# inai17ibar/video-diffusion-pipeline-parallel

Hardware: AMD Instinct MI355X
Metric: steady-state videos/sec (whole node), SVD 14f x 25step (higher is better)
Workload: dtype f16

## Files before the change

### include/svdpipe.h

```cpp
#ifndef SVDPIPE_H
#define SVDPIPE_H

#include <stddef.h>
#include <stdint.h>

#ifdef __cplusplus
extern "C" {
#endif

#define SP_OK 0
#define SP_EINVAL (-1)
#define SP_ELAUNCH (-2)

const char *sp_last_error(void);
int sp_version(void);
#define SP_ZERO_PAGE_BYTES 4096

enum { SP_A_LINEAR = 0, SP_A_CONV3X3 = 1, SP_A_TEMPORAL3 = 2 };

typedef struct sp_gemm_desc {
  const void *a;
  int64_t lda;
  int mode;
  int cin;
// ... 20 lines not shown
  float euler_sigma, euler_sigma_next;
  int euler_frames; int64_t euler_hw;
  void *workspace; size_t workspace_bytes;
  float *ln_out; float ln_out_eps;
  int64_t w_group_rows; int64_t w_group_stride;
  float *gn_part;
  const void *a2; int64_t lda2; int cin2;
  int64_t euler_guidance_ld;
} sp_gemm_desc;

int sp_gemm_f16(const sp_gemm_desc *desc, void *stream);
size_t sp_gemm_desc_size(void);
size_t sp_gemm_workspace_bytes(const sp_gemm_desc *desc);

const char *sp_gemm_last_kernel(void);

int sp_gemm_set_route(int route, int bm, int bn);

int sp_gemv_f16(const void *x, int64_t ldx, const void *w, const float *b, float *y, void *y_f16,
                int64_t ldy, int rows, int n, int k, int silu_in, int silu_out, void *stream);
int sp_gemv_batched_f16(const void *x, int64_t ldx, int64_t x_stride, const void *w, int64_t w_stride,
                        const float *b, int64_t b_stride, float *y, void *y_f16, int64_t ldy, int64_t y_stride,
                        int batch, int rows, int n, int k, int silu_in, int silu_out, void *stream);

int sp_sinusoid_f16(const float *values, void *out, int count, int dim, void *stream);

size_t sp_groupnorm_ws_bytes(int instances, int64_t rows, int c, int groups);
int sp_groupnorm_f16(const void *x, const float *gamma, const float *beta, void *y, int instances,
                     int64_t rows, int c, int groups, float eps, int fuse_silu, void *ws,
                     size_t ws_bytes, void *stream);
// ... 107 lines not shown
```

### video-diffusion-pipeline-parallel_amd/csrc/gemm.hip

```cpp
#include <cstring>
#include "gemm_args.h"
#include <stdlib.h>

using namespace spgemm;

namespace {


template <int BM, int BN, int WM, int WN, int STAGES>
__global__ __launch_bounds__(WM *WN * 64, 2) void gemm_f16_kernel(const GemmArgs p) {
  constexpr int NW = WM * WN;
  constexpr int THREADS = NW * 64;
  constexpr int WTM = BM / WM, WTN = BN / WN;
  constexpr int TN = WTN / 16;
  constexpr int TM = WTM / 16;
  constexpr int A_BYTES = BM * BK * 2;
  constexpr int B_BYTES = BN * BK * 2;
  constexpr int STAGE = A_BYTES + B_BYTES;
  constexpr int A_LOADS = BM / 8 / NW;
  constexpr int B_LOADS = BN / 8 / NW;
  constexpr int L = A_LOADS + B_LOADS;
  static_assert(A_LOADS * 8 * NW == BM && B_LOADS * 8 * NW == BN, "tile rows must split evenly over waves");
  static_assert(STAGES == 2 || STAGES == 3, "2- or 3-deep ring");
  extern __shared__ __attribute__((aligned(16))) char smem[];
// ... 568 lines not shown
}

extern "C" int sp_gemm_f32out_f16(const void *a_, int64_t lda, const void *w, void *d, int m, int n, int k,
                                  const void *zero_page, void *stream) {
  SP_REQUIRE(a_ && w && d && zero_page, "sp_gemm_f32out_f16: null a/w/d/zero_page");
  SP_REQUIRE(m > 0 && n > 0 && n % 256 == 0, "sp_gemm_f32out_f16: n=%d must be a positive multiple of 256 (m=%d)", n, m);
  SP_REQUIRE(k >= 64 && k % 64 == 0, "sp_gemm_f32out_f16: k=%d must be a multiple of 64", k);
  SP_REQUIRE(lda >= k && lda % 8 == 0, "sp_gemm_f32out_f16: lda=%lld invalid", (long long)lda);
  SP_REQUIRE(((uintptr_t)d & 15) == 0, "sp_gemm_f32out_f16: d must be 16-byte aligned");
  GemmArgs a{};
  a.a = (const f16 *)a_; a.w = (const f16 *)w; a.zero = (const char *)zero_page;
  a.lda = lda; a.mode = SP_A_LINEAR; a.cin = k; a.taps = 1; a.m = m; a.n = n; a.k = k;
  a.oscale = 1.0f; a.bias2_rows = m; a.ldb2 = n;
  a.ksplit = 1; a.partial = (float *)d;
  return spgemm::launch_pp(a, 256, 256, (hipStream_t)stream);
}

extern "C" int sp_gemm_f16(const sp_gemm_desc *d, void *stream) {
  SP_REQUIRE(d != nullptr, "sp_gemm_f16: null descriptor");
  SP_REQUIRE(d->a && d->w && d->d && d->zero_page, "sp_gemm_f16: null a/w/d/zero_page");
  SP_REQUIRE(d->m > 0 && d->n > 0, "sp_gemm_f16: m,n must be positive (m=%d n=%d)", d->m, d->n);
  SP_REQUIRE(d->cin > 0 && d->cin % 64 == 0, "sp_gemm_f16: cin=%d must be a multiple of 64", d->cin);
  SP_REQUIRE(d->n % 64 == 0, "sp_gemm_f16: n=%d must be a multiple of 64", d->n);
  SP_REQUIRE(d->mode >= SP_A_LINEAR && d->mode <= SP_A_TEMPORAL3, "sp_gemm_f16: bad mode %d", d->mode);
  SP_REQUIRE(d->lda >= d->cin && d->lda % 8 == 0, "sp_gemm_f16: lda=%lld invalid", (long long)d->lda);
  const int nout_cols = d->geglu ? d->n / 2 : d->n;
  SP_REQUIRE(d->n_store >= 0 && d->n_store <= nout_cols, "sp_gemm_f16: n_store=%d must be 0 (all) or 1 ... %d output columns",
             d->n_store, nout_cols);
  const int stored_cols = d->n_store > 0 ? d->n_store : nout_cols;
  SP_REQUIRE(d->ldd >= stored_cols && (d->ldd % 8 == 0 || (d->n_store > 0 && d->n_store < 8)),
// ... 120 lines not shown
```

### video-diffusion-pipeline-parallel_amd/csrc/gemm_args.h

```cpp
#pragma once
#include "common.h"

namespace spgemm {

constexpr int BK = 64;

template <int N>
__device__ __forceinline__ void wait_vm_lgkm() {
  asm volatile("s_waitcnt vmcnt(%0) lgkmcnt(0)" ::"n"(N) : "memory");
}

struct GemmArgs {
  const f16 *a;
  const f16 *a2;
  int64_t lda2;
  int cin2;
  const f16 *w;
  const float *bias;
  const float *bias2;
  const f16 *res1;
  const f16 *res2;
  const f16 *eul_lat; f16 *eul_out; const f16 *eul_u; const float *eul_gs;
  int64_t eul_ldu, eul_hw, eul_ldg;
  int eul_frames;
// ... 7 lines not shown
  f16 *d;
  const char *zero;
  int64_t lda, ldr1, ldr2, ldd, hw, bias2_rows, ldb2;
  int64_t w_group_rows, w_group_stride;
  int mode, cin, taps;
  int n_img, hin, win, hout, wout, stride, ups;
  int frames;
  int m, n, k;
  float oscale, r1scale, r2scale;
  int geglu, n_store;
  int tiles_m, tiles_n;
  int ksplit;
  float *partial;
  int dbg;
  int stagger;
};

__device__ __forceinline__ int xcd_remap(int bid, int nwg) {
  const int q = nwg >> 3, r = nwg & 7;
  const int xcd = bid & 7;
  const int base = xcd < r ? xcd * (q + 1) : r * (q + 1) + (xcd - r) * q;
  return base + (bid >> 3);
}


void note_kernel(const char *fmt, ...);
void note_kernel_suffix(const char *suffix);

int launch_pp(GemmArgs &a, int bm, int bn, hipStream_t s);

bool ps_supported(const GemmArgs &a, int bm, int bn);
int launch_ps(GemmArgs &a, int bm, int bn, hipStream_t s);

}
```

### video-diffusion-pipeline-parallel_amd/csrc/gemm_pp.hip

```cpp
#include "gemm_args.h"
#include <stdlib.h>
#include <type_traits>

namespace spgemm {
namespace {

constexpr int PBK = 32, PNW = 8;


#ifdef SP_GEMM_EXPERIMENTS
constexpr int PP_TRACE_WGS = 16384, PP_TRACE_SLOTS = 12;
__device__ long long g_pp_trace[PP_TRACE_WGS * PP_TRACE_SLOTS];
#define PP_TRACE(slot)                                                                              \
  do {                                                                                              \
    if (threadIdx.x == 0 && blockIdx.x < PP_TRACE_WGS)                                              \
      g_pp_trace[blockIdx.x * PP_TRACE_SLOTS + (slot)] = wall_clock64();                            \
  } while (0)
#define PP_TRACE_CLK(slot)                                                                          \
  do {                                                                                              \
    if (threadIdx.x == 0 && blockIdx.x < PP_TRACE_WGS)                                              \
      g_pp_trace[blockIdx.x * PP_TRACE_SLOTS + (slot)] = (long long)__builtin_amdgcn_s_memtime();   \
  } while (0)
#else
#define PP_TRACE(slot) do {} while (0)
// ... 7 lines not shown
#endif
constexpr int pp_stages(int bm, int bn) { return bm == 128 ? 3 : (bm == 192 && bn == 256 ? SP_PP_STAGES_192_256 : 4); }

template <int N>
__device__ __forceinline__ void wait_vm() { asm volatile("s_waitcnt vmcnt(%0)" ::"n"(N) : "memory"); }

template <int L>
__device__ __forceinline__ void wait_dma(int ksteps_left) {
  if (ksteps_left >= 3) wait_vm<3 * L>();
  else if (ksteps_left == 2) wait_vm<2 * L>();
  else if (ksteps_left == 1) wait_vm<L>();
  else wait_vm<0>();
}

#define WROWS_OF(pbm, wtm) ((pbm) / (wtm))
template <int PBM, int BN, int TN, int TM, int WTN, int WTM, bool GEGLU, int NT, bool GNRES = false>
__device__ __forceinline__ void pp_epilogue(const GemmArgs &p, f32x4 (&acc)[TN][TM], char *smem, int tile_m,
                                            int tile_n, int wm, int wn, int tid, int fr, int fq) {
  constexpr int bno = GEGLU ? BN / 2 : BN;
  constexpr int cpr = bno >> 3;
  constexpr int TNO = GEGLU ? TN / 2 : TN;
  constexpr int NCH = PBM * cpr, ITERS = (NCH + NT - 1) / NT, ITERS_A = ITERS / 2;
  static_assert(cpr % 8 == 0, "chunk swizzle works on aligned groups of 8 chunks");
  const int ncols_total = GEGLU ? p.n / 2 : p.n;
  const int nstore = p.n_store > 0 ? p.n_store : ncols_total;
  const int64_t mbase = (int64_t)tile_m * PBM;

  auto res_src = [&](const f16 *res, int64_t ldr, int it) -> const f16 * {
    const int idx = tid + it * NT;
    const int r = idx / cpr, c = idx - r * cpr;
    const int64_t m = mbase + r;
    const int col = tile_n * bno + c * 8;
    const bool ok = idx < NCH && m < p.m && col + 8 <= nstore;
// ... 16 lines not shown
      if (p.bias) b = *(const f32x4 *)(p.bias + n);
#pragma unroll
      for (int j = 0; j < TM; ++j) acc[i][j] = (acc[i][j] - st[j][0] * cs) * st[j][1] + b;
      __builtin_amdgcn_sched_barrier(0);
    }
  }
  if constexpr (!GEGLU) {
    if (p.gn_part && !p.res1 && !p.res2) {
      auto row16_sum = [](float v) {
        v += __builtin_bit_cast(float, __builtin_amdgcn_mov_dpp(__builtin_bit_cast(int, v), 0xB1, 0xF, 0xF, true));
        v += __builtin_bit_cast(float, __builtin_amdgcn_mov_dpp(__builtin_bit_cast(int, v), 0x4E, 0xF, 0xF, true));
        v += __builtin_bit_cast(float, __builtin_amdgcn_mov_dpp(__builtin_bit_cast(int, v), 0x141, 0xF, 0xF, true));
        v += __builtin_bit_cast(float, __builtin_amdgcn_mov_dpp(__builtin_bit_cast(int, v), 0x140, 0xF, 0xF, true));
        return v;
      };
      float *dst = p.gn_part + (((int64_t)tile_m * WROWS_OF(PBM, WTM) + wm) * p.n + (int64_t)tile_n * BN + wn * WTN) * 2;
#pragma unroll
      for (int i = 0; i < TN; ++i) {
        f32x4 sm = {0.f, 0.f, 0.f, 0.f}, sq = {0.f, 0.f, 0.f, 0.f};
#pragma unroll
        for (int j = 0; j < TM; ++j) {
          const f32x4 v = acc[i][j] * p.oscale;
          sm += v;
          sq += v * v;
        }
#pragma unroll
        for (int r = 0; r < 4; ++r) { sm[r] = row16_sum(sm[r]); sq[r] = row16_sum(sq[r]); }
        if (fr == 0) {
          float *o = dst + (i * 16 + 4 * fq) * 2;
          *(f32x4 *)o = (f32x4){sm[0], sq[0], sm[1], sq[1]};
          *(f32x4 *)(o + 4) = (f32x4){sm[2], sq[2], sm[3], sq[3]};
// ... 91 lines not shown
        if (p.ln_part) {
          *(float2 *)(p.ln_part + ((mbase + tid) * p.tiles_n + tile_n) * 2) = make_float2(sm, sq);
        } else {
          const float inv = 1.0f / (float)bno, mean = sm * inv;
          float var = sq * inv - mean * mean;
          if (var < 0.f) var = 0.f;
          *(float2 *)(p.ln_out + (mbase + tid) * 2) = make_float2(mean, rsqrtf(var + p.ln_out_eps));
        }
      }
    }
  }
#pragma unroll
  for (int it = 0; it < ITERS; ++it) {
    const int idx = tid + it * NT;
    const int r = idx / cpr, c = idx - r * cpr;
    const int64_t m = mbase + r;
    const int col = tile_n * bno + c * 8;
    if (idx >= NCH || m >= p.m || col >= nstore) continue;
    if (col + 8 <= nstore) {
#ifdef SP_GEMM_EXPERIMENTS
      if (p.dbg & 512) __builtin_nontemporal_store(o[it], (f16x8 *)(p.d + m * p.ldd + col));
      else
#endif
      *(f16x8 *)(p.d + m * p.ldd + col) = o[it];
      if (gn_res) *(f16x8 *)(smem + r * (bno * 2) + ((c ^ (r & 7)) << 4)) = o[it];
    } else {
      for (int e = 0; e < nstore - col; ++e) {
        float f = (float)o[it][e];
        if (p.res1) f += p.r1scale * (float)p.res1[m * p.ldr1 + col + e];
        if (p.res2) f += p.r2scale * (float)p.res2[m * p.ldr2 + col + e];
        p.d[m * p.ldd + col + e] = (f16)f;
      }
    }
// ... 67 lines not shown
            glds16(bptr[pc - NAP], dsb + (pc - NAP) * (NWV * 1024));
            bptr[pc - NAP] += PBK;
          }
        }
      }
    }
  }
}
#endif

template <int BM, int BN, int EXP>
__global__ __launch_bounds__(BM == 128 ? 256 : 512, 2) void gemm_pp_kernel(const GemmArgs p) {
  constexpr int PBM = BM;
  constexpr bool SPLITK = (EXP & 128) != 0;
  constexpr bool A2 = (EXP & 4096) != 0;
  constexpr int NWV = BM == 128 ? 4 : 8, NT = NWV * 64, WROWS = NWV / 4;
  constexpr int PSTAGES = pp_stages(BM, BN), PDIST = PSTAGES - 1;
  constexpr int TN = BN / 4 / 16;
  constexpr int TM = BM / WROWS / 16;
  constexpr int WTN = BN / 4, WTM = BM / WROWS;
  constexpr int A_BYTES = PBM * 64, B_BYTES = BN * 64, STAGE = A_BYTES + B_BYTES;
  constexpr int A_PIECES = BM / 16, B_PIECES = BN / 16;
  constexpr int A_LOADS = (A_PIECES + NWV - 1) / NWV, A_LOADS_HI = A_PIECES / NWV;
  constexpr int A_SPLIT = A_PIECES % NWV == 0 ? NWV : A_PIECES % NWV;
  constexpr int B_LOADS_LO = (B_PIECES + NWV - 1) / NWV;
  constexpr int B_LOADS_HI = B_PIECES / NWV;
  constexpr int B_SPLIT = B_PIECES % NWV == 0 ? NWV : B_PIECES % NWV;
  static_assert((B_SPLIT == NWV || B_SPLIT == 4) && (A_SPLIT == NWV || A_SPLIT == 4), "wave halves must have uniform DMA counts");
#ifdef SP_GEMM_EXPERIMENTS
  constexpr bool HALO_COUNT = (EXP & 16) != 0;
// ... 23 lines not shown
    g_pp_trace[blockIdx.x * PP_TRACE_SLOTS + 5] = ((long long)xcc << 32) | hw;
  }
#endif

  constexpr int GM = BM == 128 ? 8 : 4;
  const int nwg = p.tiles_m * p.tiles_n;
  int bid = blockIdx.x, kslice = 0;
  if constexpr (SPLITK) { kslice = bid / nwg; bid -= kslice * nwg; }
  const int t = xcd_remap(bid, nwg);
  const int per_group = GM * p.tiles_n;
  const int group = t / per_group;
  const int first_m = group * GM;
  const int gsz = min(p.tiles_m - first_m, GM);
  const int in_group = t - group * per_group;
  const int tile_n = in_group / gsz;
  const int tile_m = first_m + (in_group - tile_n * gsz);

  const int lrow = lane >> 2, lchunk = lane & 3;
  const int cpt = p.cin >> 5;

  int a_i0[A_LOADS], a_i1[A_LOADS], a_i2[A_LOADS];
  bool a_in[A_LOADS];
  int schunk_a[A_LOADS];
#pragma unroll
  for (int i = 0; i < A_LOADS; ++i) {
    const int r = (i * NWV + wave) * 16 + lrow;
    const int m = tile_m * PBM + r;
    a_in[i] = m < p.m && r < PBM;
    schunk_a[i] = (lchunk ^ swz4(r)) * 8;
    if (p.mode == SP_A_CONV3X3) {
      const int per_img = p.hout * p.wout;
      const int img = m / per_img;
      const int rem = m - img * per_img;
      const int oy = rem / p.wout;
      a_i0[i] = img;
      a_i1[i] = oy * p.stride - 1;
      a_i2[i] = (rem - oy * p.wout) * p.stride - 1;
    } else if (p.mode == SP_A_TEMPORAL3) {
      a_i0[i] = (int)((m / p.hw) % p.frames);
      a_i1[i] = 0;
      a_i2[i] = m;
    } else {
      a_i0[i] = a_i1[i] = 0;
      a_i2[i] = m;
    }
// ... 10 lines not shown
          if (a_in[i]) {
            aptr[i] = p.a2 + ((int64_t)tile_m * PBM + r) * p.lda2 + schunk_a[i];
            astep[i] = PBK;
          } else {
            aptr[i] = (const f16 *)(p.zero + lchunk * 16);
            astep[i] = 0;
          }
          continue;
        }
      }
#ifdef SP_GEMM_EXPERIMENTS
      if (a_in[i] && !((EXP & 8) && tap > 0)) {
#else
      if (a_in[i]) {
#endif
        if (p.mode == SP_A_CONV3X3) {
          const int ky = tap / 3, kx = tap - ky * 3;
          const int iy = a_i1[i] + ky, ix = a_i2[i] + kx;
          const int hv = p.hin << p.ups, wv = p.win << p.ups;
          if (iy >= 0 && iy < hv && ix >= 0 && ix < wv)
            row = ((int64_t)a_i0[i] * p.hin + (iy >> p.ups)) * p.win + (ix >> p.ups);
        } else if (p.mode == SP_A_TEMPORAL3) {
          const int f = a_i0[i] + tap - 1;
          if (f >= 0 && f < p.frames) row = (int64_t)a_i2[i] + (int64_t)(tap - 1) * p.hw;
        } else {
          row = a_i2[i];
        }
      }
      if (row >= 0) {
        aptr[i] = p.a + row * p.lda + schunk_a[i];
        astep[i] = PBK;
      } else {
        aptr[i] = (const f16 *)(p.zero + lchunk * 16);
        astep[i] = 0;
      }
    }
  };

  const f16 *bptr[B_LOADS_LO];
#pragma unroll
  for (int j = 0; j < B_LOADS_LO; ++j) {
    const int piece = j * NWV + wave;
    const int r = piece * 16 + lrow;
    const int n = tile_n * BN + (r < BN ? r : 0);
    bptr[j] = p.w + (int64_t)n * p.k + (lchunk ^ swz4(r)) * 8;
    if (p.w_group_rows > 0) bptr[j] += ((int64_t)tile_m * PBM / p.w_group_rows) * p.w_group_stride;
  }

  bool skip_a = false;
  auto stage = [&](int slot) {
    char *sa = smem + slot * STAGE;
    char *sb = sa + A_BYTES;
#pragma unroll
    for (int i = 0; i < A_LOADS; ++i) {
      if ((i < A_LOADS_HI || wave < A_SPLIT) && !skip_a) {
        glds16(aptr[i], sa + (i * NWV + wave) * 1024);
        aptr[i] += astep[i];
      }
    }
#pragma unroll
    for (int j = 0; j < B_LOADS_LO; ++j) {
// ... 39 lines not shown
  tap = kbeg / cpt;
  in_tap = kbeg - tap * cpt;
  set_tap(tap);
  if (kbeg) {
#pragma unroll
    for (int i = 0; i < A_LOADS; ++i) aptr[i] += in_tap * astep[i];
#pragma unroll
    for (int j = 0; j < B_LOADS_LO; ++j) bptr[j] += (int64_t)kbeg * PBK;
  }
  PP_TRACE(10);
#pragma unroll
  for (int s = 0; s < PDIST; ++s)
    if (s < nk) stage_next();
  PP_TRACE(11);
  __builtin_amdgcn_sched_barrier(0);
  if (p.bias2 && !SPLITK) {
    int brow[TM];
#pragma unroll
    for (int j = 0; j < TM; ++j) {
      const int m = tile_m * PBM + wm * WTM + j * 16 + fr;
      brow[j] = m < p.m ? m / (int)p.bias2_rows : 0;
    }
#pragma unroll
    for (int i = 0; i < TN; ++i) {
      const int n = tile_n * BN + wn * WTN + i * 16 + 4 * fq;
#pragma unroll
      for (int j = 0; j < TM; ++j) acc[i][j] = *(const f32x4 *)(p.bias2 + (int64_t)brow[j] * p.ldb2 + n) + bias_v[i];
      __builtin_amdgcn_sched_barrier(0);
    }
  } else {
#pragma unroll
// ... 114 lines not shown
  if (!late) __builtin_amdgcn_s_barrier();
  PP_TRACE_CLK(9);
  PP_TRACE(2);

  if constexpr (SPLITK) {
    float *slab = p.partial + (int64_t)kslice * p.m * p.n;
#pragma unroll
    for (int j = 0; j < TM; ++j) {
      const int64_t m = (int64_t)tile_m * PBM + wm * WTM + j * 16 + fr;
      if (m < p.m) {
#pragma unroll
        for (int i = 0; i < TN; ++i)
          *(f32x4 *)(slab + m * p.n + tile_n * BN + wn * WTN + i * 16 + 4 * fq) = acc[i][j];
      }
    }
  } else if (p.geglu) {
    if constexpr (TN % 2 == 0) pp_epilogue<PBM, BN, TN, TM, WTN, WTM, true, NT>(p, acc, smem, tile_m, tile_n, wm, wn, tid, fr, fq);
  } else {
    pp_epilogue<PBM, BN, TN, TM, WTN, WTM, false, NT, (EXP & 2048) != 0>(p, acc, smem, tile_m, tile_n, wm, wn, tid, fr, fq);
  }
  PP_TRACE(3);
}

template <int BM, int BN, int EXP = 0>
int launch_pp(GemmArgs &a, hipStream_t s) {
  constexpr int NSTG = pp_stages(BM, BN);
  constexpr size_t ring = (size_t)NSTG * (BM + BN) * 64, tile = (size_t)BM * BN * 2;
  constexpr size_t lds = ring > tile ? ring : tile;
  static_assert(lds <= 160 * 1024, "LDS per workgroup");
  static bool attr_set[SP_MAX_DEVICES] = {};
  if (int rc = sp_ensure_dyn_lds((const void *)gemm_pp_kernel<BM, BN, EXP>, (int)lds, attr_set, "sp_gemm_f16(pp)"))
    return rc;
  a.tiles_m = (a.m + BM - 1) / BM;
  a.tiles_n = a.n / BN;
  note_kernel((EXP & 128) ? "gemm_pp_kernel<%d, %d, %d> + splitk_reduce_kernel" : "gemm_pp_kernel<%d, %d, %d>", BM, BN, EXP);
  SP_CLEAR_STALE_ERROR();
  hipLaunchKernelGGL((gemm_pp_kernel<BM, BN, EXP>), dim3(a.tiles_m * a.tiles_n * ((EXP & 128) ? a.ksplit : 1)),
                     dim3(BM == 128 ? 256 : 512), lds, s, a);
  SP_CHECK_LAUNCH("sp_gemm_f16(pp)");
  return SP_OK;
}

}

int launch_pp(GemmArgs &a, int bm, int bn, hipStream_t s) {
  if (a.ksplit >= 1 && a.partial) return launch_pp<256, 256, 128>(a, s);
  if (a.gn_part && (a.res1 || a.res2)) return bn == 256 ? launch_pp<256, 256, 2048>(a, s) : launch_pp<256, 320, 2048>(a, s);
  if (a.a2) return bn == 256 ? launch_pp<256, 256, 4096>(a, s) : launch_pp<256, 320, 4096>(a, s);
#ifdef SP_GEMM_EXPERIMENTS
  if (bm == 256 && bn == 256) switch (a.dbg) {
    case 1: return launch_pp<256, 256, 1>(a, s);
    case 2: return launch_pp<256, 256, 2>(a, s);
    case 3: return launch_pp<256, 256, 3>(a, s);
    case 65: return launch_pp<256, 256, 65>(a, s);
    case 67: return launch_pp<256, 256, 67>(a, s);
    case 4: return launch_pp<256, 256, 4>(a, s);
    default: break;
// ... 34 lines not shown
```

### video-diffusion-pipeline-parallel_amd/hip/__init__.py

```python

from __future__ import annotations

import ctypes
import os

_HERE = os.path.dirname(os.path.abspath(__file__))
LIB_PATH = os.path.join(_HERE, "libsvdpipe_hip.so")
_lib = None


class GemmDesc(ctypes.Structure):

    _fields_ = [
        ("a", ctypes.c_void_p), ("lda", ctypes.c_int64), ("mode", ctypes.c_int), ("cin", ctypes.c_int),
        ("n_img", ctypes.c_int), ("hin", ctypes.c_int), ("win", ctypes.c_int), ("hout", ctypes.c_int),
        ("wout", ctypes.c_int), ("stride", ctypes.c_int), ("upsample2x", ctypes.c_int),
        ("frames", ctypes.c_int), ("hw", ctypes.c_int64),
        ("w", ctypes.c_void_p), ("m", ctypes.c_int), ("n", ctypes.c_int),
        ("bias", ctypes.c_void_p), ("bias2", ctypes.c_void_p), ("bias2_rows", ctypes.c_int64),
        ("ldb2", ctypes.c_int64),
        ("res1", ctypes.c_void_p), ("ldr1", ctypes.c_int64), ("r1scale", ctypes.c_float),
        ("res2", ctypes.c_void_p), ("ldr2", ctypes.c_int64), ("r2scale", ctypes.c_float),
        ("oscale", ctypes.c_float), ("geglu", ctypes.c_int), ("n_store", ctypes.c_int),
        ("d", ctypes.c_void_p), ("ldd", ctypes.c_int64), ("zero_page", ctypes.c_void_p),
# ... 9 lines not shown
        ("gn_part", ctypes.c_void_p),
        ("a2", ctypes.c_void_p), ("lda2", ctypes.c_int64), ("cin2", ctypes.c_int),
        ("euler_guidance_ld", ctypes.c_int64),
    ]


_P, _I, _L, _F, _Z = ctypes.c_void_p, ctypes.c_int, ctypes.c_int64, ctypes.c_float, ctypes.c_size_t
SIGNATURES = {
    "sp_last_error": (ctypes.c_char_p, []),
    "sp_version": (_I, []),
    "sp_gemm_f16": (_I, [ctypes.POINTER(GemmDesc), _P]),
    "sp_gemm_desc_size": (_Z, []),
    "sp_gemm_workspace_bytes": (_Z, [ctypes.POINTER(GemmDesc)]),
    "sp_gemm_set_route": (_I, [_I, _I, _I]),
    "sp_gemm_last_kernel": (ctypes.c_char_p, []),
    "sp_gemv_f16": (_I, [_P, _L, _P, _P, _P, _P, _L, _I, _I, _I, _I, _I, _P]),
    "sp_gemv_batched_f16": (_I, [_P, _L, _L, _P, _L, _P, _L, _P, _P, _L, _L, _I, _I, _I, _I, _I, _I, _P]),
    "sp_sinusoid_f16": (_I, [_P, _P, _I, _I, _P]),
    "sp_groupnorm_ws_bytes": (_Z, [_I, _L, _I, _I]),
    "sp_groupnorm_f16": (_I, [_P, _P, _P, _P, _I, _L, _I, _I, _F, _I, _P, _Z, _P]),
    "sp_groupnorm_ld_f16": (_I, [_P, _L, _P, _P, _P, _I, _L, _I, _I, _F, _I, _P, _Z, _P]),
    "sp_groupnorm_tile_sums_f16": (_I, [_P, _L, _P, _P, _P, _P, _I, _L, _I, _I, _F, _I, _P, _P]),
    "sp_groupnorm_tile_sums2_f16": (_I, [_P, _L, _P, _I, _P, _P, _P, _P, _I, _L, _I, _I, _F, _I, _P, _P]),
    "sp_groupnorm_fold_linear_tile_sums_f16": (_I, [_P, _P, _P, _I, _L, _I, _I, _F, _P, _P, _I, _P, _P, _P, _P]),
    "sp_groupnorm_fold_linear_f16": (_I, [_P, _L, _P, _P, _I, _L, _I, _I, _F, _P, _P, _I, _P, _P, _P, _Z, _P]),
    "sp_layernorm_f16": (_I, [_P, _P, _L, _P, _P, _P, _P, _L, _I, _F, _P]),
    "sp_ln_stats_f16": (_I, [_P, _P, _L, _P, _P, _L, _I, _F, _P]),
    "sp_attn_spatial_f16": (_I, [_P, _P, _P, _P, _L, _L, _L, _L, _I, _I, _I, _F, _P, _P]),
    "sp_attn_long_ws_bytes": (_L, [_I, _I, _I]),
    "sp_attn_spatial_long_f16": (_I, [_P, _P, _P, _P, _L, _L, _L, _L, _I, _I, _I, _F, _P, _P, _L, _P]),
# ... 65 lines not shown
```

### video-diffusion-pipeline-parallel_amd/hip/ops.py

```python

from __future__ import annotations

import ctypes

import torch

from . import GemmDesc, last_error, load

A_LINEAR, A_CONV3X3, A_TEMPORAL3 = 0, 1, 2
ZERO_PAGE_BYTES = 4096
_zero_pages: dict = {}


class HipKernelError(RuntimeError):
    pass


PROFILE = None


class _Timed:
    def __init__(self, kind, flops, nbytes=0.0, tag=None):
        self.kind, self.flops, self.nbytes, self.tag = kind, flops, nbytes, tag

# ... 39 lines not shown
        raise ValueError(f"{name} must be row-major (innermost stride 1); got strides {tuple(t.stride())}")
    return t


def _rows(t: torch.Tensor, name: str, ld: int) -> torch.Tensor:
    _f16(t, name)
    if t.dim() == 2 and t.shape[0] > 1 and t.stride(0) != ld:
        raise ValueError(f"{name}: row stride {t.stride(0)} does not match leading dimension {ld}")
    return t


def gemm(a, w, out, *, m, n, cin, mode=A_LINEAR, lda=None, conv=None, temporal=None, bias=None,
         bias2=None, bias2_rows=0, ldb2=0, res1=None, r1scale=1.0, res2=None, r2scale=1.0, oscale=1.0,
         geglu=False, n_store=0, ldd=None, ldr1=None, ldr2=None, ln_stats=None, ln_colsum=None, euler=None,
         workspace=None, ln_out=None, ln_out_eps=1e-5, w_group_rows=0, w_group_stride=0, gn_part=None, a2=None, cin2=0,
         lda2=None):
    d = GemmDesc()
    d.lda = int(lda if lda is not None else cin)
    d.a, d.mode, d.cin = _rows(a, "a", d.lda).data_ptr(), mode, cin
    if mode == A_CONV3X3:
        d.n_img, d.hin, d.win, d.hout, d.wout, d.stride, d.upsample2x = conv
    if mode == A_TEMPORAL3:
        d.frames, d.hw = temporal
    d.w, d.m, d.n = _f16(w, "w").data_ptr(), m, n
    d.bias, d.bias2, d.bias2_rows, d.ldb2 = _ptr(bias), _ptr(bias2), bias2_rows, ldb2
    nout = n // 2 if geglu else n
    d.res1, d.ldr1, d.r1scale = _ptr(res1), int(ldr1 if ldr1 is not None else nout), r1scale
    d.res2, d.ldr2, d.r2scale = _ptr(res2), int(ldr2 if ldr2 is not None else nout), r2scale
    d.oscale, d.geglu, d.n_store = oscale, int(geglu), n_store
    d.ldd = int(ldd if ldd is not None else (n_store or nout))
    d.d = _rows(out, "out", d.ldd).data_ptr()
# ... 19 lines not shown
    if gn_part is not None:
        if gn_part.dtype != torch.float32 or not gn_part.is_cuda or gn_part.numel() < (m // 256) * 2 * n * 2:
            raise TypeError("gn_part must be a float32 HIP tensor of (m/256)*2*n*2 elements")
        d.gn_part = gn_part.data_ptr()
    taps = 9 if mode == A_CONV3X3 else 3 if mode == A_TEMPORAL3 else 1
    a_rows = d.n_img * d.hin * d.win if mode == A_CONV3X3 else m
    k2 = int(cin2) if a2 is not None else 0
    nbytes = 2.0 * (a_rows * cin + m * k2 + n * (taps * cin + k2) + m * (n_store or nout) * (1 + (res1 is not None) + (res2 is not None)))
    with _Timed("gemm", 2.0 * m * n * (taps * cin + k2), nbytes, (m, n, cin, mode, bool(geglu))) as tm:
        _check(load().sp_gemm_f16(ctypes.byref(d), _stream()), "sp_gemm_f16")
        if PROFILE is not None:
            tm.tag = tm.tag + (load().sp_gemm_last_kernel().decode(),)
    return out


def gemm_workspace_bytes(*, m, n, cin, mode=A_LINEAR) -> int:
    d = GemmDesc()
    d.m, d.n, d.cin, d.mode = m, n, cin, mode
    return int(load().sp_gemm_workspace_bytes(ctypes.byref(d)))


class gemm_route:

    def __init__(self, route: int, bm: int = 0, bn: int = 0):
        self.args = (route, bm, bn)

    def __enter__(self):
        _check(load().sp_gemm_set_route(*self.args), "sp_gemm_set_route")
        return self

# ... 449 lines not shown
```

### video-diffusion-pipeline-parallel_amd/models/unet_hip.py

```python

from __future__ import annotations

import os
from dataclasses import dataclass

import torch

from ..hip import ops
from . import common
from . import weights as W
from .common import _Act, _Dense, _Norm, _f32
from .unet_spec import UNetConfig, up_block_plan


@dataclass
class _Run:
    b: int
    f: int
    h: int
    w: int
    temb: torch.Tensor
    ctx16: torch.Tensor
    gn_ws: torch.Tensor
    sk_ws: torch.Tensor
# ... 40 lines not shown
class SVDUNetHIP:
    FP8_MIN_SEQ = 1024
    SPLITK_MAX_ROWS = 6144
    LONG_ATTENTION_MIN_SEQ = 8192

    def __init__(self, cfg: UNetConfig, state_dict: dict, device, *, fp8_attention: bool | None = None,
                 long_attention: bool | None = None):
        self.cfg = cfg
        self.fp8_attention = (os.environ.get("VDPP_FP8_ATTN") == "1") if fp8_attention is None else bool(fp8_attention)
        self.long_attention = (os.environ.get("VDPP_LONG_ATTN", "1") != "0") if long_attention is None else bool(long_attention)
        self.fold_groupnorm = os.environ.get("VDPP_FOLD_GN", "1") != "0"
        self.gn_from_epilogue = os.environ.get("VDPP_GN_EPILOGUE", "1") != "0"
        self.gn_epilogue_residual = os.environ.get("VDPP_GN_EPILOGUE_RES", "1") != "0"
        self.fold_shortcut = os.environ.get("VDPP_FOLD_SHORTCUT", "1") != "0"
        self.ln_out_wide = os.environ.get("VDPP_LN_OUT_WIDE", "1") != "0"
        self.device = dev = common.hip_device(device, "SVDUNetHIP")
        sd = state_dict
        self._temb_w, self._temb_b, self._temb_n = [], [], 0
        self._xf_all = []
        boc = list(cfg.block_out_channels)
        g = cfg.norm_groups

        self.conv_in = _Dense.conv3x3(sd, "conv_in", dev)
        self.cin_pad = self.conv_in.cin
        self.te1 = _Dense.linear(sd, "time_embedding.linear_1", dev)
        self.ae1 = _Dense.linear(sd, "add_embedding.linear_1", dev)
        w2 = torch.cat([sd["time_embedding.linear_2.weight"], sd["add_embedding.linear_2.weight"]], dim=1)
        self.emb2_w = W.pack_linear(w2).to(dev)
        self.emb2_b = _f32(sd["time_embedding.linear_2.bias"].float() + sd["add_embedding.linear_2.bias"].float(), dev)

# ... 11 lines not shown
            ch = cout
        self.mid = (self._resblock(sd, "mid_block.resnets.0", ch, ch, 1e-5),
                    self._transformer(sd, "mid_block.attentions.0", ch),
                    self._resblock(sd, "mid_block.resnets.1", ch, ch, 1e-5))
        self.up = []
        layers = cfg.layers_per_block + 1
        for i, (in_ch, out_ch, prev, attn, _h, ups) in enumerate(up_block_plan(cfg)):
            res, att = [], []
            for j in range(layers):
                skip = in_ch if j == layers - 1 else out_ch
                rin = prev if j == 0 else out_ch
                res.append(dict(self._resblock(sd, f"up_blocks.{i}.resnets.{j}", rin + skip, out_ch, 1e-6), cx=rin))
                if attn:
                    att.append(self._transformer(sd, f"up_blocks.{i}.attentions.{j}", out_ch))
            us = _Dense.conv3x3(sd, f"up_blocks.{i}.upsamplers.0.conv", dev) if ups else None
            self.up.append((res, att, us))
        self.norm_out = _Norm(sd, "conv_norm_out", dev, 1e-5)
        self.conv_out = _Dense.conv3x3(sd, "conv_out", dev)

        self.temb_w = torch.cat(self._temb_w, dim=0).contiguous()
        self.temb_b = torch.cat(self._temb_b, dim=0).contiguous()
        del self._temb_w, self._temb_b
        self._group_small_gemvs()
        self._gn_ws = None
        self._sk_ws = {}
        self._pos_cache = {}
        self._fp8_ws = {}
        self._long_ws = {}

    def release_stream_state(self) -> None:
# ... 125 lines not shown
            t_fi1=self._geglu_ln(sd, t + ".ff_in.net.0.proj", dev, t + ".norm_in"),
            t_fi2=_Dense.linear(sd, t + ".ff_in.net.2", dev),
            t_attn=self._attn(sd, t + ".attn1", dev, t + ".norm1"),
            t_x=self._xattn(sd, t + ".attn2", dev),
            t_ff1=self._geglu_ln(sd, t + ".ff.net.0.proj", dev, t + ".norm3"),
            t_ff2=_Dense.linear(sd, t + ".ff.net.2", dev),
        )

    def _buf(self, rows, c):
        return torch.empty((rows, c), dtype=torch.float16, device=self.device)

    def _gemm(self, r: _Run, layer: _Dense, a, *, m=None, conv=None, ln_next=None, ln_out=None, **kw) -> _Act:
        m = r.m if m is None else m
        out = kw.pop("out", None)
        w_groups = kw.pop("w_groups", None)
        weight, bias = layer.w, layer.bias
        if w_groups is not None:
            weight, bias = w_groups[0], None
            kw.update(bias2=w_groups[1], bias2_rows=w_groups[2], w_group_rows=w_groups[2],
                      w_group_stride=w_groups[0].shape[1] * w_groups[0].shape[2])
        ws = r.sk_ws if m <= self.SPLITK_MAX_ROWS else None
        gn_part = None
        if kw.pop("gn_next", False) and self.gn_from_epilogue and m % 256 == 0 and layer.n == layer.n_true \
                and not layer.geglu and (layer.n % 320 == 0 or layer.n % 256 == 0) and r.hw % 256 == 0 \
                and layer.colsum is None and ln_next is None and "euler" not in kw and w_groups is None \
                and (self.gn_epilogue_residual or (kw.get("res1") is None and kw.get("res2") is None)):
            gn_part = torch.empty((m // 256, 2, layer.n, 2), dtype=torch.float32, device=self.device)
            kw.update(gn_part=gn_part)
        st = ln_out
        if st is None and ln_next is not None and self._ln_out_ok(layer, m) and "euler" not in kw:
            st = torch.empty((m, 2), dtype=torch.float32, device=self.device)
# ... 35 lines not shown

    def _gn(self, r: _Run, norm: _Norm, a: _Act, *, temporal: bool, silu: bool):
        x, c, groups = a.t, a.t.shape[1], self.cfg.norm_groups
        inst, rows = (r.b, r.f * r.hw) if temporal else (r.b * r.f, r.hw)
        y = self._buf(x.shape[0], c)
        if a.gn_part is not None and rows % 256 == 0:
            stats = torch.empty((inst, groups, 2), dtype=torch.float32, device=self.device)
            cat = dict(part_b=a.gn_part_b, c_a=a.c_a) if a.gn_part_b is not None else {}
            ops.groupnorm_tile_sums(x, a.gn_part, norm.g, norm.b, y, instances=inst, rows=rows, c=c, groups=groups,
                                    eps=norm.eps, silu=silu, stats=stats, ldx=x.stride(0), **cat)
            return y
        ops.groupnorm(x, norm.g, norm.b, y, instances=inst, rows=rows, c=c, groups=groups,
                      eps=norm.eps, silu=silu, ws=r.gn_ws, ldx=x.stride(0))
        return y

    def _conv_geom(self, r: _Run, stride=1, ups=0):
        hv, wv = r.h << ups, r.w << ups
        ho, wo = (hv - 1) // stride + 1, (wv - 1) // stride + 1
        return (r.b * r.f, r.h, r.w, ho, wo, stride, ups), ho, wo

    def _run_resblock(self, r: _Run, p, x: _Act, out=None, gn_next=False) -> _Act:
        geom, _, _ = self._conv_geom(r)
        t = self._gn(r, p["n1"], x, temporal=False, silu=True)
        t = self._gemm(r, p["c1"], t, conv=geom, **self._temb(r, p["te_s"], p["c1"].n), gn_next=True)
        t = self._gn(r, p["n2"], t, temporal=False, silu=True)
        x = x.t
        if p["sc"] is not None and p["c2sc"] is not None and self.fold_shortcut and r.m > self.SPLITK_MAX_ROWS \
                and r.m % 256 == 0:
            s = self._gemm(r, p["c2sc"], t, conv=geom, a2=x, cin2=p["c2sc"].cin2, lda2=x.stride(0), gn_next=True)
        else:
# ... 185 lines not shown
        for res, att, us in self.up:
            for j, p in enumerate(res):
                cat = skips.pop()
                last = j == len(res) - 1 and us is not None
                if att:
                    x = self._run_resblock(r, p, cat, gn_next=True)
                    x = skips.left(self._run_transformer(r, att[j], x, out=None if last else skips.left_dest(),
                                                         gn_next=not last))
                else:
                    x = skips.left(self._run_resblock(r, p, cat, out=None if last else skips.left_dest(), gn_next=not last))
                del cat
            if us is not None:
                geom, ho, wo = self._conv_geom(r, ups=1)
                m_up = r.b * r.f * ho * wo
                r.h, r.w = ho, wo
                x = skips.left(self._gemm(r, us, x.t, m=m_up, conv=geom, out=skips.left_dest(), gn_next=True))
        x = self._gn(r, self.norm_out, x, temporal=False, silu=True)
        geom, _, _ = self._conv_geom(r)
        if euler is not None:
            self._gemm(r, self.conv_out, x, conv=geom, euler=dict(euler, frames=r.f, hw=r.hw))
            return None
        return self._gemm(r, self.conv_out, x, conv=geom).t

    def __call__(self, sample, timestep, encoder_hidden_states, added_time_ids, return_dict=False, per_video=False):
        b, f, c, h, w = sample.shape
        dev = self.device
        rows = torch.zeros((b * f * h * w, self.cin_pad), dtype=torch.float16, device=dev)
        rows[:, :c] = sample.to(dev, torch.float16).permute(0, 1, 3, 4, 2).reshape(-1, c)
        t = torch.as_tensor(timestep, dtype=torch.float32).reshape(-1)
        t_differ = t.numel() > 1 and bool((t != t[0]).any())
        if t.numel() not in (1, b) or (t_differ and not per_video):
# ... 20 lines not shown
```

### video-diffusion-pipeline-parallel_amd/models/weights.py

```python

from __future__ import annotations

import torch


def round_up(v: int, m: int) -> int:
    return (v + m - 1) // m * m


def pack_conv3x3(w: torch.Tensor, cin_pad: int | None = None, n_pad: int | None = None) -> torch.Tensor:
    cout, cin = w.shape[:2]
    cp = cin_pad or round_up(cin, 64)
    npad = n_pad or round_up(cout, 64)
    out = torch.zeros(npad, 9, cp, dtype=torch.float16, device=w.device)
    out[:cout, :, :cin] = w.permute(0, 2, 3, 1).reshape(cout, 9, cin).to(torch.float16)
    return out.reshape(npad, 9 * cp).contiguous()


def pack_tconv3(w: torch.Tensor) -> torch.Tensor:
    cout, cin = w.shape[:2]
    return w[:, :, :, 0, 0].permute(0, 2, 1).reshape(cout, 3 * cin).to(torch.float16).contiguous()


def pack_linear(w: torch.Tensor) -> torch.Tensor:
    return w.reshape(w.shape[0], -1).to(torch.float16).contiguous()


def interleave_geglu(w: torch.Tensor, b: torch.Tensor | None):
    two_inner = w.shape[0]
    inner = two_inner // 2
    assert inner % 16 == 0
# ... 6 lines not shown
```

Before: 0.8198.

## Fold nearest-upsample into 3x3 conv as four 2x2 phase convolutions

Adds a phase-decomposed upsampler path. A nearest-2x upsample followed by a 3x3 conv is rewritten as four 2x2 convolutions, one per output phase, each reading the low-resolution input directly. Folded weights are packed per phase, and the GEMM kernel gains an UP variant that remaps input taps, output rows and GroupNorm partial-sum slots. This cuts the multiply count from 9 taps to 4 per output pixel. The cost is extra weight memory and a new kernel specialisation, plus a heuristic that falls back when the group-norm partial layout does not fit.

```diff
diff --git a/include/svdpipe.h b/include/svdpipe.h
--- a/include/svdpipe.h
+++ b/include/svdpipe.h
@@ -58,6 +58,9 @@
 size_t sp_gemm_workspace_bytes(const sp_gemm_desc *desc);
 
 const char *sp_gemm_last_kernel(void);
+
+int sp_conv_up2x_f16(const void *a, int64_t lda, int cin, int n_img, int hin, int win, const void *w, int n,
+                     const float *bias, void *d, int64_t ldd, float *gn_part, const void *zero_page, void *stream);
 
 int sp_gemm_set_route(int route, int bm, int bn);
 
diff --git a/video-diffusion-pipeline-parallel_amd/csrc/gemm.hip b/video-diffusion-pipeline-parallel_amd/csrc/gemm.hip
--- a/video-diffusion-pipeline-parallel_amd/csrc/gemm.hip
+++ b/video-diffusion-pipeline-parallel_amd/csrc/gemm.hip
@@ -606,6 +606,36 @@
   a.oscale = 1.0f; a.bias2_rows = m; a.ldb2 = n;
   a.ksplit = 1; a.partial = (float *)d;
   return spgemm::launch_pp(a, 256, 256, (hipStream_t)stream);
+}
+
+extern "C" int sp_conv_up2x_f16(const void *a_, int64_t lda, int cin, int n_img, int hin, int win, const void *w, int n,
+                                const float *bias, void *d, int64_t ldd, float *gn_part, const void *zero_page, void *stream) {
+  SP_REQUIRE(a_ && w && d && zero_page, "sp_conv_up2x_f16: null a/w/d/zero_page");
+  SP_REQUIRE((((uintptr_t)a_ | (uintptr_t)w | (uintptr_t)d | (uintptr_t)zero_page | (uintptr_t)bias | (uintptr_t)gn_part) & 15) == 0,
+             "sp_conv_up2x_f16: a, w, d, zero_page, bias and gn_part must be 16-byte aligned");
+  SP_REQUIRE(cin > 0 && cin % 64 == 0, "sp_conv_up2x_f16: cin=%d must be a positive multiple of 64", cin);
+  SP_REQUIRE(n > 0 && (n % 256 == 0 || n % 320 == 0), "sp_conv_up2x_f16: n=%d must be a positive multiple of 256 or 320", n);
+  SP_REQUIRE(lda >= cin && lda % 8 == 0, "sp_conv_up2x_f16: lda=%lld must be >= cin (%d) and a multiple of 8", (long long)lda, cin);
+  SP_REQUIRE(ldd >= n && ldd % 8 == 0, "sp_conv_up2x_f16: ldd=%lld must be >= n (%d) and a multiple of 8", (long long)ldd, n);
+  SP_REQUIRE(n_img > 0 && hin > 0 && win > 0, "sp_conv_up2x_f16: geometry (n_img=%d, hin=%d, win=%d) must be positive", n_img,
+             hin, win);
+  const int64_t rows = (int64_t)n_img * hin * win;
+  SP_REQUIRE(4 * rows <= 0x7fffffff, "sp_conv_up2x_f16: n_img*hin*win=%lld: the 4x as many output rows must fit an int",
+             (long long)rows);
+  SP_REQUIRE(!gn_part || ((int64_t)hin * win) % 256 == 0,
+             "sp_conv_up2x_f16: gn_part needs frames of whole 256-row tiles per phase (hin*win = %lld)", (long long)hin * win);
+  GemmArgs a{};
+  a.a = (const f16 *)a_; a.w = (const f16 *)w; a.bias = bias; a.d = (f16 *)d; a.zero = (const char *)zero_page;
+  a.gn_part = gn_part;
+  a.lda = lda; a.ldd = ldd;
+  a.mode = SP_A_CONV3X3; a.cin = cin; a.taps = 4;
+  a.n_img = n_img; a.hin = hin; a.win = win; a.hout = 2 * hin; a.wout = 2 * win; a.stride = 1; a.ups = 1;
+  a.m = (int)rows; a.n = n; a.k = 4 * cin;
+  a.oscale = 1.0f; a.r1scale = 1.0f; a.r2scale = 1.0f;
+  a.bias2_rows = a.m; a.ldb2 = n;
+  a.up_tiles = (a.m + 255) / 256;
+  a.up_gn_tiles = gn_part ? hin * win / 256 : 1;
+  return spgemm::launch_pp_up2x(a, n % 320 == 0 ? 320 : 256, (hipStream_t)stream);
 }
 
 extern "C" int sp_gemm_f16(const sp_gemm_desc *d, void *stream) {
diff --git a/video-diffusion-pipeline-parallel_amd/csrc/gemm_args.h b/video-diffusion-pipeline-parallel_amd/csrc/gemm_args.h
--- a/video-diffusion-pipeline-parallel_amd/csrc/gemm_args.h
+++ b/video-diffusion-pipeline-parallel_amd/csrc/gemm_args.h
@@ -45,6 +45,8 @@
   float *partial;
   int dbg;
   int stagger;
+  int up_tiles;
+  int up_gn_tiles;
 };
 
 __device__ __forceinline__ int xcd_remap(int bid, int nwg) {
@@ -59,6 +61,7 @@
 void note_kernel_suffix(const char *suffix);
 
 int launch_pp(GemmArgs &a, int bm, int bn, hipStream_t s);
+int launch_pp_up2x(GemmArgs &a, int bn, hipStream_t s);
 
 bool ps_supported(const GemmArgs &a, int bm, int bn);
 int launch_ps(GemmArgs &a, int bm, int bn, hipStream_t s);
diff --git a/video-diffusion-pipeline-parallel_amd/csrc/gemm_pp.hip b/video-diffusion-pipeline-parallel_amd/csrc/gemm_pp.hip
--- a/video-diffusion-pipeline-parallel_amd/csrc/gemm_pp.hip
+++ b/video-diffusion-pipeline-parallel_amd/csrc/gemm_pp.hip
@@ -45,9 +45,9 @@
 }
 
 #define WROWS_OF(pbm, wtm) ((pbm) / (wtm))
-template <int PBM, int BN, int TN, int TM, int WTN, int WTM, bool GEGLU, int NT, bool GNRES = false>
+template <int PBM, int BN, int TN, int TM, int WTN, int WTM, bool GEGLU, int NT, bool GNRES = false, bool UP = false>
 __device__ __forceinline__ void pp_epilogue(const GemmArgs &p, f32x4 (&acc)[TN][TM], char *smem, int tile_m,
-                                            int tile_n, int wm, int wn, int tid, int fr, int fq) {
+                                            int tile_n, int wm, int wn, int tid, int fr, int fq, int phase = 0) {
   constexpr int bno = GEGLU ? BN / 2 : BN;
   constexpr int cpr = bno >> 3;
   constexpr int TNO = GEGLU ? TN / 2 : TN;
@@ -94,7 +94,12 @@
         v += __builtin_bit_cast(float, __builtin_amdgcn_mov_dpp(__builtin_bit_cast(int, v), 0x140, 0xF, 0xF, true));
         return v;
       };
-      float *dst = p.gn_part + (((int64_t)tile_m * WROWS_OF(PBM, WTM) + wm) * p.n + (int64_t)tile_n * BN + wn * WTN) * 2;
+      int gn_tile = tile_m;
+      if constexpr (UP) {
+        const int frame = tile_m / p.up_gn_tiles;
+        gn_tile = (frame * 4 + phase) * p.up_gn_tiles + (tile_m - frame * p.up_gn_tiles);
+      }
+      float *dst = p.gn_part + (((int64_t)gn_tile * WROWS_OF(PBM, WTM) + wm) * p.n + (int64_t)tile_n * BN + wn * WTN) * 2;
 #pragma unroll
       for (int i = 0; i < TN; ++i) {
         f32x4 sm = {0.f, 0.f, 0.f, 0.f}, sq = {0.f, 0.f, 0.f, 0.f};
@@ -216,9 +221,15 @@
   for (int it = 0; it < ITERS; ++it) {
     const int idx = tid + it * NT;
     const int r = idx / cpr, c = idx - r * cpr;
-    const int64_t m = mbase + r;
+    int64_t m = mbase + r;
     const int col = tile_n * bno + c * 8;
     if (idx >= NCH || m >= p.m || col >= nstore) continue;
+    if constexpr (UP) {
+      const int mi = (int)m, per_img = p.hin * p.win;
+      const int img = mi / per_img, rem = mi - img * per_img;
+      const int sy = rem / p.win, sx = rem - sy * p.win;
+      m = ((int64_t)img * (2 * p.hin) + 2 * sy + (phase >> 1)) * (2 * p.win) + 2 * sx + (phase & 1);
+    }
     if (col + 8 <= nstore) {
 #ifdef SP_GEMM_EXPERIMENTS
       if (p.dbg & 512) __builtin_nontemporal_store(o[it], (f16x8 *)(p.d + m * p.ldd + col));
@@ -316,6 +327,7 @@
   constexpr int PBM = BM;
   constexpr bool SPLITK = (EXP & 128) != 0;
   constexpr bool A2 = (EXP & 4096) != 0;
+  constexpr bool UP = (EXP & 8192) != 0;
   constexpr int NWV = BM == 128 ? 4 : 8, NT = NWV * 64, WROWS = NWV / 4;
   constexpr int PSTAGES = pp_stages(BM, BN), PDIST = PSTAGES - 1;
   constexpr int TN = BN / 4 / 16;
@@ -369,7 +381,9 @@
   const int gsz = min(p.tiles_m - first_m, GM);
   const int in_group = t - group * per_group;
   const int tile_n = in_group / gsz;
-  const int tile_m = first_m + (in_group - tile_n * gsz);
+  const int tile_mg = first_m + (in_group - tile_n * gsz);
+  const int phase = UP ? tile_mg / p.up_tiles : 0;
+  const int tile_m = UP ? tile_mg - phase * p.up_tiles : tile_mg;
 
   const int lrow = lane >> 2, lchunk = lane & 3;
   const int cpt = p.cin >> 5;
@@ -383,7 +397,15 @@
     const int m = tile_m * PBM + r;
     a_in[i] = m < p.m && r < PBM;
     schunk_a[i] = (lchunk ^ swz4(r)) * 8;
-    if (p.mode == SP_A_CONV3X3) {
+    if constexpr (UP) {
+      const int per_img = p.hin * p.win;
+      const int img = m / per_img;
+      const int rem = m - img * per_img;
+      const int sy = rem / p.win;
+      a_i0[i] = img;
+      a_i1[i] = sy + (phase >> 1) - 1;
+      a_i2[i] = (rem - sy * p.win) + (phase & 1) - 1;
+    } else if (p.mode == SP_A_CONV3X3) {
       const int per_img = p.hout * p.wout;
       const int img = m / per_img;
       const int rem = m - img * per_img;
@@ -424,7 +446,10 @@
 #else
       if (a_in[i]) {
 #endif
-        if (p.mode == SP_A_CONV3X3) {
+        if constexpr (UP) {
+          const int iy = a_i1[i] + (tap >> 1), ix = a_i2[i] + (tap & 1);
+          if (iy >= 0 && iy < p.hin && ix >= 0 && ix < p.win) row = ((int64_t)a_i0[i] * p.hin + iy) * p.win + ix;
+        } else if (p.mode == SP_A_CONV3X3) {
           const int ky = tap / 3, kx = tap - ky * 3;
           const int iy = a_i1[i] + ky, ix = a_i2[i] + kx;
           const int hv = p.hin << p.ups, wv = p.win << p.ups;
@@ -455,6 +480,7 @@
     const int n = tile_n * BN + (r < BN ? r : 0);
     bptr[j] = p.w + (int64_t)n * p.k + (lchunk ^ swz4(r)) * 8;
     if (p.w_group_rows > 0) bptr[j] += ((int64_t)tile_m * PBM / p.w_group_rows) * p.w_group_stride;
+    if constexpr (UP) bptr[j] += (int64_t)phase * p.n * p.k;
   }
 
   bool skip_a = false;
@@ -524,7 +550,7 @@
     if (s < nk) stage_next();
   PP_TRACE(11);
   __builtin_amdgcn_sched_barrier(0);
-  if (p.bias2 && !SPLITK) {
+  if (!UP && p.bias2 && !SPLITK) {
     int brow[TM];
 #pragma unroll
     for (int j = 0; j < TM; ++j) {
@@ -669,10 +695,11 @@
           *(f32x4 *)(slab + m * p.n + tile_n * BN + wn * WTN + i * 16 + 4 * fq) = acc[i][j];
       }
     }
-  } else if (p.geglu) {
+  } else if (!UP && p.geglu) {
     if constexpr (TN % 2 == 0) pp_epilogue<PBM, BN, TN, TM, WTN, WTM, true, NT>(p, acc, smem, tile_m, tile_n, wm, wn, tid, fr, fq);
   } else {
-    pp_epilogue<PBM, BN, TN, TM, WTN, WTM, false, NT, (EXP & 2048) != 0>(p, acc, smem, tile_m, tile_n, wm, wn, tid, fr, fq);
+    pp_epilogue<PBM, BN, TN, TM, WTN, WTM, false, NT, (EXP & 2048) != 0, UP>(p, acc, smem, tile_m, tile_n, wm, wn, tid, fr, fq,
+                                                                             phase);
   }
   PP_TRACE(3);
 }
@@ -686,7 +713,7 @@
   static bool attr_set[SP_MAX_DEVICES] = {};
   if (int rc = sp_ensure_dyn_lds((const void *)gemm_pp_kernel<BM, BN, EXP>, (int)lds, attr_set, "sp_gemm_f16(pp)"))
     return rc;
-  a.tiles_m = (a.m + BM - 1) / BM;
+  a.tiles_m = (EXP & 8192) ? 4 * a.up_tiles : (a.m + BM - 1) / BM;
   a.tiles_n = a.n / BN;
   note_kernel((EXP & 128) ? "gemm_pp_kernel<%d, %d, %d> + splitk_reduce_kernel" : "gemm_pp_kernel<%d, %d, %d>", BM, BN, EXP);
   SP_CLEAR_STALE_ERROR();
@@ -696,6 +723,10 @@
   return SP_OK;
 }
 
+}
+
+int launch_pp_up2x(GemmArgs &a, int bn, hipStream_t s) {
+  return bn == 256 ? launch_pp<256, 256, 8192>(a, s) : launch_pp<256, 320, 8192>(a, s);
 }
 
 int launch_pp(GemmArgs &a, int bm, int bn, hipStream_t s) {
diff --git a/video-diffusion-pipeline-parallel_amd/hip/__init__.py b/video-diffusion-pipeline-parallel_amd/hip/__init__.py
--- a/video-diffusion-pipeline-parallel_amd/hip/__init__.py
+++ b/video-diffusion-pipeline-parallel_amd/hip/__init__.py
@@ -47,6 +47,7 @@
     "sp_gemm_workspace_bytes": (_Z, [ctypes.POINTER(GemmDesc)]),
     "sp_gemm_set_route": (_I, [_I, _I, _I]),
     "sp_gemm_last_kernel": (ctypes.c_char_p, []),
+    "sp_conv_up2x_f16": (_I, [_P, _L, _I, _I, _I, _I, _P, _I, _P, _P, _L, _P, _P, _P]),
     "sp_gemv_f16": (_I, [_P, _L, _P, _P, _P, _P, _L, _I, _I, _I, _I, _I, _P]),
     "sp_gemv_batched_f16": (_I, [_P, _L, _L, _P, _L, _P, _L, _P, _P, _L, _L, _I, _I, _I, _I, _I, _I, _P]),
     "sp_sinusoid_f16": (_I, [_P, _P, _I, _I, _P]),
diff --git a/video-diffusion-pipeline-parallel_amd/hip/ops.py b/video-diffusion-pipeline-parallel_amd/hip/ops.py
--- a/video-diffusion-pipeline-parallel_amd/hip/ops.py
+++ b/video-diffusion-pipeline-parallel_amd/hip/ops.py
@@ -77,7 +77,16 @@
          bias2=None, bias2_rows=0, ldb2=0, res1=None, r1scale=1.0, res2=None, r2scale=1.0, oscale=1.0,
          geglu=False, n_store=0, ldd=None, ldr1=None, ldr2=None, ln_stats=None, ln_colsum=None, euler=None,
          workspace=None, ln_out=None, ln_out_eps=1e-5, w_group_rows=0, w_group_stride=0, gn_part=None, a2=None, cin2=0,
-         lda2=None):
+         lda2=None, up2x_phases=False):
+    if up2x_phases:
+        refused = dict(temporal=(temporal, None), bias2=(bias2, None), res1=(res1, None), res2=(res2, None),
+                       ln_stats=(ln_stats, None), ln_colsum=(ln_colsum, None), euler=(euler, None), ln_out=(ln_out, None),
+                       a2=(a2, None), geglu=(bool(geglu), False), n_store=(n_store, 0), w_group_rows=(w_group_rows, 0),
+                       oscale=(oscale, 1.0))
+        extra = sorted(k for k, (v, neutral) in refused.items() if (v is not None if neutral is None else v != neutral))
+        if extra:
+            raise ValueError(f"gemm(up2x_phases=True) takes a bias only; got {', '.join(extra)}")
+        return _conv_up2x(a, w, out, m=m, n=n, cin=cin, mode=mode, lda=lda, conv=conv, bias=bias, ldd=ldd, gn_part=gn_part)
     d = GemmDesc()
     d.lda = int(lda if lda is not None else cin)
     d.a, d.mode, d.cin = _rows(a, "a", d.lda).data_ptr(), mode, cin
@@ -127,6 +136,30 @@
     return out
 
 
+def _conv_up2x(a, w, out, *, m, n, cin, mode, lda, conv, bias, ldd, gn_part):
+    if mode != A_CONV3X3 or conv is None or conv[-1] != 1 or conv[5] != 1:
+        raise ValueError("gemm(up2x_phases=True) needs mode=A_CONV3X3 and an upsampling geometry (stride 1, upsample2x = 1)")
+    n_img, hin, win, hout, wout = conv[:5]
+    if (hout, wout) != (2 * hin, 2 * win) or m != n_img * hout * wout:
+        raise ValueError(f"gemm(up2x_phases=True): m = {m}, output {hout}x{wout} do not match {n_img} images of {hin}x{win} doubled")
+    if tuple(_f16(w, "w").shape) != (4, n, 4 * cin) or not w.is_contiguous():
+        raise ValueError(f"gemm(up2x_phases=True): w must be the contiguous phase-major pack [4][{n}][{4 * cin}]; got {tuple(w.shape)}")
+    lda = int(lda if lda is not None else cin)
+    ldd = int(ldd if ldd is not None else n)
+    _rows(a, "a", lda)
+    _rows(out, "out", ldd)
+    if gn_part is not None:
+        if gn_part.dtype != torch.float32 or not gn_part.is_cuda or gn_part.numel() < (m // 256) * 2 * n * 2:
+            raise TypeError("gn_part must be a float32 HIP tensor of (m/256)*2*n*2 elements")
+    nbytes = 2.0 * (n_img * hin * win * cin + n * 16 * cin + m * n)
+    with _Timed("gemm", 2.0 * m * n * 4 * cin, nbytes, (m, n, cin, mode, False)) as tm:
+        _check(load().sp_conv_up2x_f16(a.data_ptr(), lda, cin, n_img, hin, win, w.data_ptr(), n, _ptr(bias), out.data_ptr(),
+                                       ldd, _ptr(gn_part), zero_page(a.device).data_ptr(), _stream()), "sp_conv_up2x_f16")
+        if PROFILE is not None:
+            tm.tag = tm.tag + (load().sp_gemm_last_kernel().decode(),)
+    return out
+
+
 def gemm_workspace_bytes(*, m, n, cin, mode=A_LINEAR) -> int:
     d = GemmDesc()
     d.m, d.n, d.cin, d.mode = m, n, cin, mode
diff --git a/video-diffusion-pipeline-parallel_amd/models/unet_hip.py b/video-diffusion-pipeline-parallel_amd/models/unet_hip.py
--- a/video-diffusion-pipeline-parallel_amd/models/unet_hip.py
+++ b/video-diffusion-pipeline-parallel_amd/models/unet_hip.py
@@ -78,6 +78,7 @@
         self.gn_epilogue_residual = os.environ.get("VDPP_GN_EPILOGUE_RES", "1") != "0"
         self.fold_shortcut = os.environ.get("VDPP_FOLD_SHORTCUT", "1") != "0"
         self.ln_out_wide = os.environ.get("VDPP_LN_OUT_WIDE", "1") != "0"
+        self.upsample_phases = os.environ.get("VDPP_UPSAMPLE_PHASES", "1") != "0"
         self.device = dev = common.hip_device(device, "SVDUNetHIP")
         sd = state_dict
         self._temb_w, self._temb_b, self._temb_n = [], [], 0
@@ -119,6 +120,8 @@
                 if attn:
                     att.append(self._transformer(sd, f"up_blocks.{i}.attentions.{j}", out_ch))
             us = _Dense.conv3x3(sd, f"up_blocks.{i}.upsamplers.0.conv", dev) if ups else None
+            if us is not None and us.n == us.n_true and (us.n % 256 == 0 or us.n % 320 == 0):
+                us.w_up2x = W.pack_conv3x3_up2x(sd[f"up_blocks.{i}.upsamplers.0.conv.weight"].to(dev), us.cin, us.n)
             self.up.append((res, att, us))
         self.norm_out = _Norm(sd, "conv_norm_out", dev, 1e-5)
         self.conv_out = _Dense.conv3x3(sd, "conv_out", dev)
@@ -274,7 +277,7 @@
         m = r.m if m is None else m
         out = kw.pop("out", None)
         w_groups = kw.pop("w_groups", None)
-        weight, bias = layer.w, layer.bias
+        weight, bias = kw.pop("weight", layer.w), layer.bias
         if w_groups is not None:
             weight, bias = w_groups[0], None
             kw.update(bias2=w_groups[1], bias2_rows=w_groups[2], w_group_rows=w_groups[2],
@@ -340,6 +343,19 @@
                       eps=norm.eps, silu=silu, ws=r.gn_ws, ldx=x.stride(0))
         return y
 
+    def _upsample_plan(self, us: _Dense, n_img, hin, win):
+        hout, wout = 2 * hin, 2 * win
+        m_out = n_img * hout * wout
+        nine_tap_sums = (hout * wout) % 256 == 0 and m_out % 256 == 0
+        if not self.upsample_phases or getattr(us, "w_up2x", None) is None:
+            return False, True
+        if nine_tap_sums and (hin * win) % 256 != 0:
+            saved = 10.0 * m_out * us.n * us.cin / 1e15
+            stats_pass = 10e-6 + 2.0 * m_out * us.n / 4e12
+            if saved < 2.0 * stats_pass:
+                return False, True
+        return True, (hin * win) % 256 == 0
+
     def _conv_geom(self, r: _Run, stride=1, ups=0):
         hv, wv = r.h << ups, r.w << ups
         ho, wo = (hv - 1) // stride + 1, (wv - 1) // stride + 1
@@ -555,7 +571,9 @@
                 geom, ho, wo = self._conv_geom(r, ups=1)
                 m_up = r.b * r.f * ho * wo
                 r.h, r.w = ho, wo
-                x = skips.left(self._gemm(r, us, x.t, m=m_up, conv=geom, out=skips.left_dest(), gn_next=True))
+                phases, sums = self._upsample_plan(us, *geom[:3])
+                up = dict(up2x_phases=True, weight=us.w_up2x) if phases else {}
+                x = skips.left(self._gemm(r, us, x.t, m=m_up, conv=geom, out=skips.left_dest(), gn_next=sums, **up))
         x = self._gn(r, self.norm_out, x, temporal=False, silu=True)
         geom, _, _ = self._conv_geom(r)
         if euler is not None:
diff --git a/video-diffusion-pipeline-parallel_amd/models/weights.py b/video-diffusion-pipeline-parallel_amd/models/weights.py
--- a/video-diffusion-pipeline-parallel_amd/models/weights.py
+++ b/video-diffusion-pipeline-parallel_amd/models/weights.py
@@ -15,6 +15,28 @@
     out = torch.zeros(npad, 9, cp, dtype=torch.float16, device=w.device)
     out[:cout, :, :cin] = w.permute(0, 2, 3, 1).reshape(cout, 9, cin).to(torch.float16)
     return out.reshape(npad, 9 * cp).contiguous()
+
+
+def fold_conv3x3_up2x(w: torch.Tensor) -> torch.Tensor:
+    rows = (lambda k: (k[0], k[1] + k[2]), lambda k: (k[0] + k[1], k[2]))
+    wt = w.permute(2, 3, 0, 1)
+    out = w.new_zeros((4, 2, 2) + tuple(wt.shape[2:]))
+    for py in range(2):
+        wy = rows[py](wt)
+        for px in range(2):
+            for ty in range(2):
+                wx = rows[px](wy[ty])
+                out[2 * py + px, ty, 0], out[2 * py + px, ty, 1] = wx[0], wx[1]
+    return out.permute(0, 3, 1, 2, 4).contiguous()
+
+
+def pack_conv3x3_up2x(w: torch.Tensor, cin_pad: int | None = None, n_pad: int | None = None) -> torch.Tensor:
+    cout, cin = w.shape[:2]
+    cp = cin_pad or round_up(cin, 64)
+    npad = n_pad or round_up(cout, 64)
+    out = torch.zeros(4, npad, 4, cp, dtype=torch.float16, device=w.device)
+    out[:, :cout, :, :cin] = fold_conv3x3_up2x(w.float()).reshape(4, cout, 4, cin).to(torch.float16)
+    return out.reshape(4, npad, 4 * cp).contiguous()
 
 
 def pack_tconv3(w: torch.Tensor) -> torch.Tensor:
```

Result: faster. 0.8319 (median of 6 runs) (+1.5%).
